# Russoul/cuda-mat

Hardware: AMD Instinct MI355X
Metric: BiCGSTAB iters/sec + SpMV effective HBM GB/s, 10M-row CSR at 1/2/4/8 GPUs (higher is better)
Workload: dtype f64

## Files before the change

cuda_mat_amd/csrc/spmv_pb.h:

```cpp
#pragma once
#include "kernels.h"
#include "valdict.h"

namespace cm {

constexpr int kPbMaxChunks = 16;

struct PbCols {
    int64_t per = 0;
    int chunks = 1;
    int rank = 0;
};

struct PbPlan {
    int n = 0;
    int64_t n_cols = 0;
    int64_t nnz = 0;
    int CB = 0, NCB = 0;
    int64_t per = 0;
    int chunks = 1;
    int64_t chunk_len = 0;
    int bpc = 0;
    int RB = 0, NRB = 0;
    int NW = 0;
    int SR = 0;
    int LPS = 64;
    int depth = 4;
    int NSUB = 0;
    double *pv = nullptr;
    unsigned char *pvi = nullptr;
    const double *dict = nullptr;
    int ndict = 0;
    unsigned short *pc = nullptr;
    unsigned short *pr = nullptr;
    double *P = nullptr;
    int *cstart = nullptr;
    int *col0 = nullptr;
    int *sstart = nullptr;
    int *slen = nullptr;
    int *order = nullptr;
    int part_off[kPbMaxChunks + 2] = {0};
    int placed = -1;
    int place_slabs = 0;
    double place_seconds = 0.0;
    float place_check_ms = 0.f, place_fast_ms = 0.f, place_slow_ms = 0.f;
    char place_classes[192] = {0};
    bool pc_zeroed = false;
    double build_seconds = 0.0;
};

struct PbCut {
    int per, chunks, chunk_len, bpc, CB;
};
struct PbBuild {
    PbPlan p;
    int *bins = nullptr;
    PbCut cut{};
    size_t cap = 0;
    double t0 = 0.0;
    bool verbose = false;
    bool two_pass = false;
    int place = 0;
    bool report_classes = false;
    double place_max_seconds = 0.3;
    int fill_occ = 0;
    int GB = 1, NG = 1;
    unsigned long long *smeta = nullptr;
    int *gstart = nullptr;
};
int pb_build_begin(hipStream_t st, const Config &cfg, int n, int64_t n_cols, int64_t nnz, const int *rp, const int *ci,
                   const PbCols *cols, PbBuild *b);
int pb_build_alloc(hipStream_t st, const Config &cfg, int n, int64_t n_cols, int64_t nnz, const PbCols *cols, PbBuild *b);
int pb_build_count(hipStream_t st, const Config &cfg, const int *rp, const int *ci, PbBuild *b);
int pb_build_values(hipStream_t st, PbBuild *b, const ValDict *vd);
int pb_build_fill(hipStream_t st, PbBuild *b, const int *rp, const int *ci, const double *val, const ValDict *vd, int sub0, int sub1);
int pb_build_end(hipStream_t st, PbBuild *b, PbPlan *out);
void pb_build_abort(PbBuild *b);

bool pb_candidate(hipStream_t st, int n, int64_t n_cols, int64_t nnz, const int *rp, const int *ci);
int pb_build(hipStream_t st, const Config &cfg, int n, int64_t n_cols, int64_t nnz, const int *rp, const int *ci,
             const double *val, PbPlan *out, const PbCols *cols = nullptr, const ValDict *vd = nullptr);
void pb_free(PbPlan *p);
int pb_strict_for(cudamat_ctx *ctx, int *strict);
int launch_spmv_pb(hipStream_t st, const PbPlan &plan, const SpmvArgs &a);
int launch_pb_check(hipStream_t st, const SpmvArgs &a);
int launch_pb_phase1(hipStream_t st, const PbPlan &plan, const SpmvArgs &a, int part);
int launch_pb_phase2(hipStream_t st, const PbPlan &plan, const SpmvArgs &a);

}
```

cuda_mat_amd/csrc/spmv_pb.hip:

```cpp
#include <algorithm>
#include <map>
#include <mutex>
#include <string>
#include <vector>

#include "device.h"
#include "spmv_pb.h"

namespace cm {

typedef unsigned short u16;
constexpr int kPbBuildWaves = 4;
constexpr int kP1Threads = 1024;
constexpr int kP1Unroll = 8;
constexpr int kTileMax = 13312;
constexpr int kPbAlign = 64;

void pb_free(PbPlan *p)
{
    void *ptrs[] = {p->pv, p->pvi, p->pc, p->pr, p->P, p->cstart, p->col0, p->sstart, p->slen, p->order};
    for (void *q : ptrs)
        if (q) CM_DROP(hipFree(q));
    *p = PbPlan();
}

bool pb_candidate(hipStream_t st, int n, int64_t n_cols, int64_t nnz, const int *rp, const int *ci)
{
    (void)st; (void)rp; (void)ci;
    if (n < 65536 || nnz < (1 << 20) || n_cols * 8 < (1 << 20)) return false;
    if ((double)nnz / n < 4.0) return false;
    if ((int64_t)n > (int64_t)kMaxParts * kTileMax) return false;
    return true;
}

__device__ __forceinline__ int col_to_cb(const PbCut &c, int col)
{
    const int q = col / c.per, w = col - q * c.per;
    const int ch = w / c.chunk_len, off = w - ch * c.chunk_len;
    return (q * c.chunks + ch) * c.bpc + off / c.CB;
}

__device__ __forceinline__ int col_to_cb_fast(const PbCut &c, double inv_cb, int col)
{
    if (c.chunks == 1 && col < c.per) {
        int cb = (int)((double)col * inv_cb);
        cb -= (long long)cb * c.CB > (long long)col ? 1 : 0;
        cb += (long long)(cb + 1) * c.CB <= (long long)col ? 1 : 0;
        return cb;
    }
    return col_to_cb(c, col);
}

__device__ __forceinline__ int wave_match_rank(unsigned long long *tab, int key, bool active, int lane, int nkeys, int *count_of_key_lane)
{
    if (lane < nkeys) tab[lane] = 0ULL;
    __builtin_amdgcn_fence(__ATOMIC_RELEASE, "wavefront");
    __builtin_amdgcn_wave_barrier();
    if (active) atomicOr(&tab[key], 1ULL << lane);
    __builtin_amdgcn_fence(__ATOMIC_RELEASE, "wavefront");
    __builtin_amdgcn_wave_barrier();
    const unsigned long long mine = active ? tab[key] : 0ULL;
    *count_of_key_lane = lane < nkeys ? __popcll(tab[lane]) : 0;
    __builtin_amdgcn_fence(__ATOMIC_RELEASE, "wavefront");
    __builtin_amdgcn_wave_barrier();
    return __popcll(mine & ((1ULL << lane) - 1ULL));
}

template <bool FILL>
__global__ __launch_bounds__(64 * kPbBuildWaves) void k_pb_rows(int n, const int *rp, const int *ci,
                                                               const double *val, PbCut cut, const int *col0, int NCB,
                                                               int SR, int NSUB, int *bins, double *pv, u16 *pc, u16 *pr,
                                                               const unsigned char *vidx, unsigned char *pvi, int sub0, int sub1)
{
    extern __shared__ int lds_i[];
    const int wave = threadIdx.x >> 6, lane = threadIdx.x & 63;
    const int sub = sub0 + blockIdx.x * kPbBuildWaves + wave;
    if (sub >= sub1) return;
    int *cur = lds_i + (size_t)wave * NCB;
    for (int c = lane; c < NCB; c += 64) cur[c] = FILL ? bins[(size_t)c * NSUB + sub] : 0;
    __builtin_amdgcn_fence(__ATOMIC_RELEASE, "wavefront");
    __builtin_amdgcn_wave_barrier();
    const long long row0 = (long long)sub * SR;
    const int row1 = (int)(row0 + SR < n ? row0 + SR : n);
    for (int row = (int)row0; row < row1; row++) {
        const int rs = rp[row], re = rp[row + 1];
        for (int k0 = rs; k0 < re; k0 += 64) {
            const int k = k0 + lane;
            const bool active = k < re;
            const int col = active ? ci[k] : -1;
            const int cb = active ? col_to_cb(cut, col) : -1;
            const int prev = __shfl_up(cb, 1, 64);
            const bool head = lane == 0 || cb != prev;
            int hs = head ? lane : 0;
#pragma unroll
            for (int o = 1; o < 64; o <<= 1) {
                const int t = __shfl_up(hs, o, 64);
                if (lane >= o) hs = t > hs ? t : hs;
            }
            const int next = __shfl_down(cb, 1, 64);
            const bool tail = lane == 63 || next != cb;
            if (active) {
                const int base = cur[cb];
                const int rank = lane - hs;
// ... 186 lines not shown
    for (int t0 = 0; t0 < len; t0 += 256) {
        unsigned m[4];
        double v[4];
        unsigned char vi[4];
        int dest[4];
#pragma unroll
        for (int u = 0; u < 4; u++) {
            const int t = t0 + 64 * u + lane;
            const bool active = t < len;
            const int loc = active ? (int)inv[t] : 0;
            m[u] = raw[loc];
            v[u] = 0.0;
            vi[u] = 0;
            if (active) { if (pvi) vi[u] = sval8[start + loc]; else v[u] = sval[start + loc]; }
            const int cbl = active ? (int)cbs[loc] : 0;
            dest[u] = __shfl(gdst, cbl, 64) + (t - __shfl(lbase, cbl, 64));
        }
#pragma unroll
        for (int u = 0; u < 4; u++) {
            if (t0 + 64 * u + lane < len) {
                if (pvi) pvi[dest[u]] = vi[u];
                else pv[dest[u]] = v[u];
                pc[dest[u]] = (u16)((m[u] >> 16) & 0xffff);
                pr[dest[u]] = (u16)(m[u] & 0xffff);
            }
        }
    }
}

__global__ __launch_bounds__(kBlock) void k_pb_colsum(int NSUB, const int *bins, int *colsum)
{
    __shared__ int red[kBlock / 64];
    const int *b = bins + (size_t)blockIdx.x * NSUB;
    int acc = 0;
    for (int i = threadIdx.x; i < NSUB; i += kBlock) acc += b[i];
#pragma unroll
    for (int o = 32; o > 0; o >>= 1) acc += __shfl_xor(acc, o, 64);
    if ((threadIdx.x & 63) == 0) red[threadIdx.x >> 6] = acc;
    __syncthreads();
    if (threadIdx.x == 0) {
        int t = 0;
        for (int w = 0; w < kBlock / 64; w++) t += red[w];
        colsum[blockIdx.x] = t;
    }
}

__global__ __launch_bounds__(kBlock) void k_pb_colscan(int NCB, const int *colsum, int *cstart, int align)
{
    __shared__ int lds_waves[kBlock / 64];
    int run = 0;
    for (int c0 = 0; c0 < NCB; c0 += kBlock) {
        const int c = c0 + threadIdx.x;
        const int v = c < NCB ? (colsum[c] + align - 1) / align * align : 0;
        int total;
        const int ex = block_scan_int(v, lds_waves, &total);
        if (c < NCB) cstart[c] = run + ex;
        run += total;
    }
    if (threadIdx.x == 0) cstart[NCB] = run;
}

__global__ __launch_bounds__(kBlock) void k_pb_segscan(int NCB, int NSUB, const int *cstart, int *bins, int *sstart,
                                                       int *slen)
{
    __shared__ int lds_waves[kBlock / 64];
    const int c = blockIdx.x;
    int *b = bins + (size_t)c * NSUB;
    int run = cstart[c];
    for (int s0 = 0; s0 < NSUB; s0 += kBlock) {
        const int sidx = s0 + threadIdx.x;
        const int cnt = sidx < NSUB ? b[sidx] : 0;
        int total;
        const int ex = block_scan_int(cnt, lds_waves, &total);
        if (sidx < NSUB) {
            const int start = run + ex;
            b[sidx] = start;
            sstart[(size_t)sidx * NCB + c] = start;
            slen[(size_t)sidx * NCB + c] = cnt;
        }
        run += total;
    }
}

static int round_blocks(int64_t n, int tile_max)
{
    int64_t m = (n + (int64_t)256 * tile_max - 1) / ((int64_t)256 * tile_max);
    if (m < 1) m = 1;
    return (int)(256 * m);
}

static void pb_scratch_free(PbBuild *b)
{
    if (b->smeta) CM_DROP(hipFree(b->smeta));
    if (b->gstart) CM_DROP(hipFree(b->gstart));
    b->smeta = nullptr;
    b->gstart = nullptr;
}

void pb_build_abort(PbBuild *b)
{
    pb_scratch_free(b);
    if (b->bins) CM_DROP(hipFree(b->bins));
    b->bins = nullptr;
    pb_free(&b->p);
}

int pb_build_begin(hipStream_t st, const Config &cfg, int n, int64_t n_cols, int64_t nnz, const int *rp, const int *ci,
                   const PbCols *cols, PbBuild *b)
{
    CM_TRY(pb_build_alloc(st, cfg, n, n_cols, nnz, cols, b));
    return pb_build_count(st, cfg, rp, ci, b);
}

int pb_build_alloc(hipStream_t st, const Config &cfg, int n, int64_t n_cols, int64_t nnz, const PbCols *cols, PbBuild *b)
{
    b->t0 = now_s();
    PbPlan &p = b->p;
    p = PbPlan();
    p.n = n;
    p.n_cols = n_cols;
    p.nnz = nnz;
    int local_slice = 0;
    if (cols && cols->per > 0 && cols->per < n_cols) {
        p.per = cols->per;
        p.chunks = cols->chunks < 1 ? 1 : cols->chunks > kPbMaxChunks ? kPbMaxChunks : cols->chunks;
        p.chunk_len = (p.per + p.chunks - 1) / p.chunks;
        p.bpc = (int)((p.chunk_len + kTileMax - 1) / kTileMax);
        p.CB = (int)((p.chunk_len + p.bpc - 1) / p.bpc);
        const int64_t slices = (n_cols + p.per - 1) / p.per;
        p.NCB = (int)(slices * p.chunks * p.bpc);
        local_slice = cols->rank;
    } else {
        p.per = n_cols;
        p.chunks = 1;
        p.chunk_len = n_cols;
        p.NCB = round_blocks(n_cols, kTileMax);
        p.CB = (int)((n_cols + p.NCB - 1) / p.NCB);
        p.NCB = (int)((n_cols + p.CB - 1) / p.CB);
        p.bpc = p.NCB;
    }
    const double seg_target = 48.0;
    double nsub_t = (double)nnz / ((double)p.NCB * seg_target);
    const bool few = nsub_t < 2560.0 && (double)n / 2048.0 * 8.0 * 8.0 <= 144.0 * 1024.0;
    double min_waves = few ? 2048.0 : 4096.0;
    if (cfg.pb_min_waves) min_waves = (double)cfg.pb_min_waves;
    if (nsub_t < min_waves) nsub_t = min_waves;
    if (nsub_t > (double)n / 16.0) nsub_t = (double)n / 16.0;
    if (nsub_t < 4.0) nsub_t = 4.0;
    p.NW = nsub_t >= 4096.0 ? 16 : nsub_t >= 2048.0 ? 8 : 4;
    int nrb = (int)(nsub_t / p.NW / 256.0 + 0.5) * 256;
    if (nrb < 256) nrb = 256;
    const int nrb_min = (int)(((int64_t)n + kTileMax - 1) / kTileMax);
    while (nrb < nrb_min) nrb += 256;
    if (nrb > kMaxParts) nrb = kMaxParts;
    p.NRB = nrb;
    p.RB = (int)(((int64_t)n + p.NRB - 1) / p.NRB);
    p.SR = (p.RB + p.NW - 1) / p.NW;
    if (p.SR < 1) p.SR = 1;
    p.RB = p.SR * p.NW;
    p.NRB = (int)(((int64_t)n + p.RB - 1) / p.RB);
    p.NSUB = p.NRB * p.NW;
    const double seg = (double)nnz / ((double)p.NCB * p.NSUB);
    p.LPS = seg <= 6.0 ? 16 : seg <= 22.0 ? 32 : 64;
    p.depth = few ? 16 : 4;
    if (cfg.pb_depth) p.depth = cfg.pb_depth;
    if (p.NRB > kMaxParts || p.CB > 65536 || p.SR > 65536 || (size_t)p.RB * 8 > 150 * 1024 ||
        sizeof(int) * (size_t)kPbBuildWaves * p.NCB > 150 * 1024) {
        set_error("pb_build: matrix shape outside the blocked kernel's limits");
        return CUDAMAT_ERR_ARG;
    }
    const size_t nbins = (size_t)p.NCB * p.NSUB;
    int *&bins = b->bins;
    bins = nullptr;
    int rc = CUDAMAT_OK;
    do {
        if ((rc = dev_alloc(&bins, nbins))) break;
        constexpr int align = kPbAlign;
        const size_t cap = (size_t)nnz + (size_t)(align - 1) * (size_t)p.NCB + 16;
        b->cap = cap;
        if ((rc = dev_alloc(&p.cstart, (size_t)p.NCB + 1))) break;
        if ((rc = dev_alloc(&p.col0, (size_t)p.NCB + 1))) break;
        if ((rc = dev_alloc(&p.order, (size_t)p.NCB))) break;
        {
            std::vector<int> h0((size_t)p.NCB + 1), ord;
            const int per_slice = p.chunks * p.bpc;
            for (int cb = 0; cb <= p.NCB; cb++) {
                const int64_t q = cb / per_slice, ch = (cb % per_slice) / p.bpc, k = cb % p.bpc;
                int64_t in_piece = k * (int64_t)p.CB;
                if (in_piece > p.chunk_len) in_piece = p.chunk_len;
                int64_t in_slice = ch * p.chunk_len + in_piece;
                if (in_slice > p.per) in_slice = p.per;
                int64_t c0 = q * p.per + in_slice;
                if (c0 > n_cols) c0 = n_cols;
                h0[(size_t)cb] = (int)c0;
            }
            ord.reserve((size_t)p.NCB);
            const int slices = p.NCB / per_slice;
            if (slices > 1) {
                for (int k = 0; k < per_slice; k++) ord.push_back(local_slice * per_slice + k);
                p.part_off[0] = 0;
                p.part_off[1] = (int)ord.size();
                for (int ch = 0; ch < p.chunks; ch++) {
                    for (int q = 0; q < slices; q++)
                        if (q != local_slice)
                            for (int k = 0; k < p.bpc; k++) ord.push_back((q * p.chunks + ch) * p.bpc + k);
                    p.part_off[ch + 2] = (int)ord.size();
                }
            } else {
                for (int cb = 0; cb < p.NCB; cb++) ord.push_back(cb);
                p.part_off[0] = 0;
                for (int ch = 0; ch <= p.chunks; ch++) p.part_off[ch + 1] = p.NCB;
            }
            if (hipMemcpyAsync(p.col0, h0.data(), sizeof(int) * h0.size(), hipMemcpyHostToDevice, st) != hipSuccess ||
                hipMemcpyAsync(p.order, ord.data(), sizeof(int) * ord.size(), hipMemcpyHostToDevice, st) != hipSuccess ||
                hipStreamSynchronize(st) != hipSuccess) { rc = CUDAMAT_ERR_HIP; set_error("pb column cut upload failed"); break; }
        }
        b->cut = PbCut{(int)p.per, p.chunks, (int)p.chunk_len, p.bpc, p.CB};
        if ((rc = dev_alloc(&p.sstart, nbins))) break;
        if ((rc = dev_alloc(&p.slen, nbins))) break;
        if ((rc = set_max_lds((const void *)k_pb_count))) break;
        if ((rc = set_max_lds((const void *)k_pb_rows<true>))) break;
        b->GB = 1;
        while (b->GB * kPbGroups < p.NCB) b->GB *= 2;
        b->NG = (p.NCB + b->GB - 1) / b->GB;
        b->fill_occ = cfg.pb_fill_occ;
        b->place = cfg.pb_place;
        b->place_max_seconds = 1e-3 * cfg.pb_place_max_ms;
        b->verbose = cfg.verbose != 0;
        b->report_classes = cfg.verbose >= 2;
        b->two_pass = cfg.pb_fill2 != 0 && nnz > 0 && nnz < 0x7fffffffLL && p.SR <= 65536 && b->GB <= 64;
        if (b->two_pass) {
            if (dev_alloc(&b->smeta, (size_t)nnz) != CUDAMAT_OK || dev_alloc(&b->gstart, (size_t)p.NSUB * (size_t)(b->NG + 1)) != CUDAMAT_OK) {
                if (b->smeta) CM_DROP(hipFree(b->smeta));
                b->smeta = nullptr;
                b->two_pass = false;
            }
        }
    } while (0);
    if (rc) pb_build_abort(b);
    return rc;
}

int pb_build_count(hipStream_t st, const Config &cfg, const int *rp, const int *ci, PbBuild *b)
{
    PbPlan &p = b->p;
    const int n = p.n;
    const int64_t nnz = p.nnz;
    int *bins = b->bins;
    constexpr int align = kPbAlign;
    int rc = CUDAMAT_OK;
    do {
        const PbCut cut = b->cut;
        const unsigned grid = (unsigned)((p.NSUB + kPbBuildWaves - 1) / kPbBuildWaves);
        const size_t lds = sizeof(int) * (size_t)kPbBuildWaves * p.NCB;
        hipLaunchKernelGGL(k_pb_count, dim3(grid), dim3(64 * kPbBuildWaves), lds, st, n, rp, ci, cut, p.NCB, p.SR, p.NSUB, bins, 0, p.NSUB);
        if (hipGetLastError() != hipSuccess) { rc = CUDAMAT_ERR_HIP; set_error("pb count launch failed"); break; }
        hipLaunchKernelGGL(k_pb_colsum, dim3(p.NCB), dim3(kBlock), 0, st, p.NSUB, bins, p.cstart);
        hipLaunchKernelGGL(k_pb_colscan, dim3(1), dim3(kBlock), 0, st, p.NCB, p.cstart, p.cstart, align);
        hipLaunchKernelGGL(k_pb_segscan, dim3(p.NCB), dim3(kBlock), 0, st, p.NCB, p.NSUB, p.cstart, bins, p.sstart, p.slen);
        int counted = -1;
        if (hipGetLastError() != hipSuccess ||
            hipMemcpyAsync(&counted, p.cstart + p.NCB, sizeof(int), hipMemcpyDeviceToHost, st) != hipSuccess ||
            hipStreamSynchronize(st) != hipSuccess) { rc = CUDAMAT_ERR_HIP; set_error("pb scan failed"); break; }
        if ((int64_t)counted < nnz || (int64_t)counted > nnz + (int64_t)(align - 1) * p.NCB) {
            rc = CUDAMAT_ERR_ARG; set_error("pb_build: counted %d entries, expected %lld", counted, (long long)nnz); break;
        }
        b->verbose = cfg.verbose != 0;
        b->report_classes = cfg.verbose >= 2;
    } while (0);
    if (rc) pb_build_abort(b);
    return rc;
}

__global__ __launch_bounds__(1024) void k_place_probe(const double2 *rd, double2 *wr, long n2)
{
    const long per = (n2 + gridDim.x - 1) / gridDim.x;
    const long lo = blockIdx.x * per, hi = lo + per < n2 ? lo + per : n2;
    for (long i = lo + threadIdx.x; i < hi; i += 1024) {
        const double2 v = rd[i];
        double2 o;
        o.x = v.x * 1.5;
        o.y = v.y + 1.0;
        wr[i] = o;
    }
}

struct PlaceTimer {
    hipStream_t st;
    hipEvent_t e0 = nullptr, e1 = nullptr;
    bool ok = false;
    int launches = 0;
    explicit PlaceTimer(hipStream_t s) : st(s) { ok = hipEventCreate(&e0) == hipSuccess && hipEventCreate(&e1) == hipSuccess; }
    ~PlaceTimer()
    {
        if (e0) CM_DROP(hipEventDestroy(e0));
        if (e1) CM_DROP(hipEventDestroy(e1));
    }
    float ms(const void *rd, void *wr, size_t bytes)
    {
        float t[12];
        int n = 0;
        while (ok && n < 12) {
            if (hipEventRecord(e0, st) != hipSuccess) { ok = false; break; }
            hipLaunchKernelGGL(k_place_probe, dim3(256), dim3(1024), 0, st, (const double2 *)rd, (double2 *)wr, (long)(bytes / 16));
            float x = 0.f;
            if (hipGetLastError() != hipSuccess || hipEventRecord(e1, st) != hipSuccess || hipEventSynchronize(e1) != hipSuccess ||
                hipEventElapsedTime(&x, e0, e1) != hipSuccess) { ok = false; break; }
            launches++;
            t[n++] = x;
            if (n >= 3) {
                const float lo = fminf(t[n - 1], fminf(t[n - 2], t[n - 3])), hi = fmaxf(t[n - 1], fmaxf(t[n - 2], t[n - 3]));
                if (hi <= 1.015f * lo) return lo;
            }
        }
        if (!ok || n < 3) return -1.f;
        return fminf(t[n - 1], fminf(t[n - 2], t[n - 3]));
    }
};

constexpr size_t kPlaceBlock = (size_t)2 << 30;
constexpr size_t kPlaceSample = (size_t)896 << 20;
constexpr size_t kPlaceSlab = (size_t)16 << 30;
constexpr size_t kPlaceMinBytes = (size_t)2 << 30;
constexpr size_t kPlaceMaxHeld = (size_t)96 << 30;
constexpr float kPlaceGap = 1.035f;

struct PlaceMemo {
    unsigned gen = ~0u;
    std::map<char *, int> cls;
    std::vector<char *> ref;
    float t_own = 0.f;
    float t_lo = 0.f, t_hi = 0.f;
    std::vector<std::pair<char *, float>> provisional;
    bool relabel = false;
    void reset() { cls.clear(); ref.clear(); provisional.clear(); t_own = t_lo = t_hi = 0.f; relabel = false; }
};
static std::mutex g_place_mu;
static std::map<int, PlaceMemo> g_place;

struct PlaceRun { size_t slab; size_t first, count; int cls; };

struct PlaceSlab {
// ... 247 lines not shown
        }
        hipLaunchKernelGGL(k_pb_group, dim3(grid), dim3(64 * kPbBuildWaves), pad, st, p.n, rp, ci, val, vidx, b->cut, p.col0, p.NCB, p.SR,
                           p.slen, b->GB, b->NG, b->gstart, p.P, p.pvi ? (unsigned char *)p.P : (unsigned char *)nullptr, b->smeta, sub0, sub1);
        const long long buckets = (long long)(sub1 - sub0) * b->NG;
        hipLaunchKernelGGL(k_pb_scatter, dim3((unsigned)((buckets + kPbScatterWaves - 1) / kPbScatterWaves)), dim3(64 * kPbScatterWaves), 0, st,
                           p.NCB, p.NSUB, p.slen, b->bins, b->GB, b->NG, b->gstart, p.P, p.pvi ? (const unsigned char *)p.P : (const unsigned char *)nullptr,
                           b->smeta, p.pv, p.pvi, p.pc, p.pr, sub0, sub1);
    } else {
        const size_t lds = sizeof(int) * (size_t)kPbBuildWaves * p.NCB;
        hipLaunchKernelGGL(k_pb_rows<true>, dim3(grid), dim3(64 * kPbBuildWaves), lds, st, p.n, rp, ci, val, b->cut, p.col0,
                           p.NCB, p.SR, p.NSUB, b->bins, p.pv, p.pc, p.pr, vidx, p.pvi, sub0, sub1);
    }
    if (hipGetLastError() != hipSuccess) { set_error("pb fill launch failed"); pb_build_abort(b); return CUDAMAT_ERR_HIP; }
    return CUDAMAT_OK;
}

static void pb_print_plan(const PbPlan &p)
{
    const size_t nbins = (size_t)p.NCB * p.NSUB;
    std::vector<int> hl(nbins);
    if (hipMemcpy(hl.data(), p.slen, sizeof(int) * nbins, hipMemcpyDeviceToHost) != hipSuccess) return;
    long long hist[7] = {0, 0, 0, 0, 0, 0, 0}, in_long = 0;
    for (int v : hl) {
        hist[v == 0 ? 0 : v <= 8 ? 1 : v <= 24 ? 2 : v <= 48 ? 3 : v <= 64 ? 4 : v <= 128 ? 5 : 6]++;
        if (v > 64) in_long += v;
    }
    fprintf(stderr, "[cudamat] pb arrays: pv %p pvi %p pc %p pr %p P %p sstart %p slen %p cstart %p\n", (void *)p.pv, (void *)p.pvi, (void *)p.pc,
            (void *)p.pr, (void *)p.P, (void *)p.sstart, (void *)p.slen, (void *)p.cstart);
    fprintf(stderr, "[cudamat] pb plan: %d x %lld, nnz %lld, NCB %d (CB %d), NSUB %d (NW %d, SR %d), LPS %d, depth %d; segments: "
                    "empty %lld, 1-8 %lld, 9-24 %lld, 25-48 %lld, 49-64 %lld, 65-128 %lld, >128 %lld; %.1f %% of the entries in "
                    "segments longer than a wave\n",
            p.n, (long long)p.n_cols, (long long)p.nnz, p.NCB, p.CB, p.NSUB, p.NW, p.SR, p.LPS, p.depth, hist[0], hist[1], hist[2], hist[3],
            hist[4], hist[5], hist[6], 100.0 * (double)in_long / (double)(p.nnz > 0 ? p.nnz : 1));
}

static void place_report_classes(hipStream_t st, const PbPlan &p, size_t cap)
{
    if (!pool_enabled()) return;
    PlaceTimer tm(st);
    if (!tm.ok) return;
    int dev = 0;
    if (hipGetDevice(&dev) != hipSuccess) return;
    std::lock_guard<std::mutex> lock(g_place_mu);
    PlaceMemo &m = g_place[dev];
    if (m.gen != pool_generation()) { m.gen = pool_generation(); m.reset(); }
    std::vector<char *> slabs;
    std::vector<char *> scratch(3, nullptr);
    for (int k = 0; k < 4 && !(scratch[0] && scratch[1] && scratch[2]); k++) {
        char *base = nullptr;
        if (hipMalloc(&base, kPlaceSlab) != hipSuccess) { CM_DROP(hipGetLastError()); break; }
        slabs.push_back(base);
        char *seg = nullptr;
        size_t bytes = 0;
        if (!pool_segment_of(base, &seg, &bytes)) break;
        char *b0 = seg + ((size_t)(base - seg) + kPlaceBlock - 1) / kPlaceBlock * kPlaceBlock;
        for (char *q = b0; q + kPlaceBlock <= base + bytes; q += kPlaceBlock) {
            const int c = place_class_of(tm, m, q);
            if (c >= 0 && c < 3 && !scratch[c]) scratch[c] = q;
        }
    }
    struct Arr { const char *name; const char *ptr; size_t bytes; };
    const Arr arrs[4] = {{"values", p.pv ? (const char *)p.pv : (const char *)p.pvi, p.pv ? sizeof(double) * cap : cap},
                         {"col idx", (const char *)p.pc, sizeof(u16) * cap}, {"row idx", (const char *)p.pr, sizeof(u16) * cap}, {"products", (const char *)p.P, sizeof(double) * cap}};
    for (const Arr &a : arrs) {
        std::string line;
        for (size_t off = 0; off + kPlaceSample <= a.bytes; off += kPlaceSample) {
            int cls = -1;
            float worst = 0.f;
            for (int k = 0; k < 3; k++) {
                if (!scratch[k]) continue;
                const float t = tm.ms(a.ptr + off, scratch[k] + kPlaceBlock - kPlaceSample, kPlaceSample);
                if (t > worst) { worst = t; cls = k; }
            }
            line += cls < 0 || !(m.t_hi >= kPlaceGap * m.t_lo) || worst <= sqrtf(m.t_lo * m.t_hi) ? '?' : (char)('0' + cls);
        }
        fprintf(stderr, "[cudamat] pb classes: %-8s at %p, per %zu MB: %s\n", a.name, (const void *)a.ptr, kPlaceSample >> 20, line.c_str());
    }
    for (char *q : slabs) CM_DROP(hipFree(q));
}

int pb_build_end(hipStream_t st, PbBuild *b, PbPlan *out)
{
    if (hipStreamSynchronize(st) != hipSuccess) { set_error("pb fill failed"); pb_build_abort(b); return CUDAMAT_ERR_HIP; }
    if (b->verbose) pb_print_plan(b->p);
    if (b->report_classes && sizeof(double) * b->cap >= kPlaceMinBytes) place_report_classes(st, b->p, b->cap);
    pb_scratch_free(b);
    CM_DROP(hipFree(b->bins));
    b->bins = nullptr;
    b->p.build_seconds = now_s() - b->t0;
    *out = b->p;
    b->p = PbPlan();
    return CUDAMAT_OK;
}

int pb_build(hipStream_t st, const Config &cfg, int n, int64_t n_cols, int64_t nnz, const int *rp, const int *ci,
             const double *val, PbPlan *out, const PbCols *cols, const ValDict *vd)
{
    PbBuild b;
    CM_TRY(pb_build_begin(st, cfg, n, n_cols, nnz, rp, ci, cols, &b));
    CM_TRY(pb_build_values(st, &b, vd));
    CM_TRY(pb_build_fill(st, &b, rp, ci, val, vd, 0, b.p.NSUB));
    return pb_build_end(st, &b, out);
}


__global__ __launch_bounds__(kP1Threads) void k_pb_phase1(const double *x, const int *col0, const int *list,
                                                          const int *cstart, const double *pv, const u16 *pc,
                                                          double *P, const LoopState *st, int cb0)
{
    extern __shared__ __attribute__((aligned(16))) double xs[];
    if (st && st->state != 0) return;
    const int cb = list ? list[blockIdx.x] : (int)blockIdx.x + cb0;
    const int s = cstart[cb], e = cstart[cb + 1];
    if (s >= e) return;
    const int c0 = col0[cb], cn = col0[cb + 1] - c0;
    for (int i = threadIdx.x; i < cn; i += kP1Threads) xs[i] = x[c0 + i];
    __syncthreads();
    constexpr int STEP = 2 * kP1Threads;
    const int k0 = (s & ~1) + 2 * (int)threadIdx.x;
    for (int k = k0; k < e; k += 4 * STEP) {
        double2 v[4];
        ushort2 c[4];
        bool full[4];
#pragma unroll
        for (int u = 0; u < 4; u++) {
            const int kk = k + u * STEP;
            full[u] = kk >= s && kk + 1 < e;
            if (full[u]) {
                v[u] = *(const double2 *)(pv + kk);
                c[u] = *(const ushort2 *)(pc + kk);
            }
        }
#pragma unroll
        for (int u = 0; u < 4; u++) {
            const int kk = k + u * STEP;
            if (full[u]) {
                double2 o;
                o.x = v[u].x * xs[c[u].x];
                o.y = v[u].y * xs[c[u].y];
                *(double2 *)(P + kk) = o;
            } else {
                if (kk >= s && kk < e) P[kk] = pv[kk] * xs[pc[kk]];
                if (kk + 1 >= s && kk + 1 < e) P[kk + 1] = pv[kk + 1] * xs[pc[kk + 1]];
            }
        }
    }
}

__global__ __launch_bounds__(kP1Threads) void k_pb_phase1_dict(const double *x, const int *col0, const int *list,
                                                               const int *cstart, const unsigned char *pvi, const u16 *pc,
                                                               const double *dict, int cb_doubles, double *P,
                                                               const LoopState *st, int cb0)
{
    extern __shared__ __attribute__((aligned(16))) double xs[];
    if (st && st->state != 0) return;
    const int cb = list ? list[blockIdx.x] : (int)blockIdx.x + cb0;
    const int s = cstart[cb], e = cstart[cb + 1];
    if (s == e) return;
    double *dv = xs + cb_doubles;
    const int c0 = col0[cb], cn = col0[cb + 1] - c0;
    for (int i = threadIdx.x; i < cn; i += kP1Threads) xs[i] = x[c0 + i];
    if (threadIdx.x < kDictMax) dv[threadIdx.x] = dict[threadIdx.x];
    __syncthreads();
    constexpr int U = kP1Unroll, STEP = 2 * kP1Threads, CH = U * STEP;
    const int a0 = (s + 1) & ~1;
    if (threadIdx.x == 0 && s < a0) P[s] = dv[pvi[s]] * xs[pc[s]];
    int kb = a0;
    const int t2 = 2 * (int)threadIdx.x;
    for (; kb + CH <= e; kb += CH) {
        const int k = kb + t2;
        u16 iv[U];
        unsigned cv[U];
#pragma unroll
        for (int u = 0; u < U; u++) {
            iv[u] = *(const u16 *)(pvi + k + u * STEP);
            cv[u] = *(const unsigned *)(pc + k + u * STEP);
        }
#pragma unroll
        for (int u = 0; u < U; u++) {
            double2 o;
            o.x = dv[iv[u] & 0xffu] * xs[cv[u] & 0xffffu];
            o.y = dv[iv[u] >> 8] * xs[cv[u] >> 16];
            *(double2 *)(P + k + u * STEP) = o;
        }
    }
    {
        const int m = e > kb ? (e - kb) / STEP : 0;
        const int k = kb + t2;
        u16 iv[U - 1];
        unsigned cv[U - 1];
#pragma unroll
        for (int u = 0; u < U - 1; u++) {
            if (u < m) {
                iv[u] = *(const u16 *)(pvi + k + u * STEP);
                cv[u] = *(const unsigned *)(pc + k + u * STEP);
            }
        }
#pragma unroll
        for (int u = 0; u < U - 1; u++) {
            if (u < m) {
                double2 o;
                o.x = dv[iv[u] & 0xffu] * xs[cv[u] & 0xffffu];
                o.y = dv[iv[u] >> 8] * xs[cv[u] >> 16];
                *(double2 *)(P + k + u * STEP) = o;
            }
        }
        const int kr = k + m * STEP;
        if (kr + 1 < e) {
            const u16 iw = *(const u16 *)(pvi + kr);
            const unsigned cw = *(const unsigned *)(pc + kr);
            double2 o;
            o.x = dv[iw & 0xffu] * xs[cw & 0xffffu];
            o.y = dv[iw >> 8] * xs[cw >> 16];
            *(double2 *)(P + kr) = o;
        } else if (kr < e) {
            P[kr] = dv[pvi[kr]] * xs[pc[kr]];
        }
    }
}

struct Pb2Args {
    int n, NCB, SR;
    const int *sstart, *slen;
    const double *P;
    const u16 *pr;
    const double *d, *xd;
    double alpha, beta;
    double *y;
    int dot;
    const double *w;
    double *parts;
    const LoopState *st;
    int strict;
    const int *xd_idx;
};

__device__ __forceinline__ void pb_seg_add(double *my, int r, double p, bool on, int lane, int group_first, bool strict)
{
    if (!strict) {
        if (on) unsafeAtomicAdd(&my[r], p);
        return;
    }
    const int r_prev = __shfl_up(r, 1, 64);
    const int on_prev = __shfl_up((int)on, 1, 64);
    const bool d1 = on && lane > group_first && on_prev && r_prev == r;
    if (on && !d1) unsafeAtomicAdd(&my[r], p);
    if (__ballot(d1) == 0) return;
    const bool d2 = d1 && __shfl_up((int)d1, 1, 64) != 0;
    if (d1 && !d2) unsafeAtomicAdd(&my[r], p);
    if (__ballot(d2) == 0) return;
    int head = d1 ? 0 : lane;
#pragma unroll
    for (int o = 1; o < 64; o <<= 1) {
        const int t = __shfl_up(head, o, 64);
        if (lane >= o) head = t > head ? t : head;
    }
    const int rank = on ? lane - head : 0;
    for (int q = 2; __ballot(on && rank >= q); q++)
        if (on && rank == q) unsafeAtomicAdd(&my[r], p);
}

__global__ __launch_bounds__(64) void k_lds_order_probe(int *mismatch)
{
    __shared__ double acc[64], val[64], start[64];
    const int lane = threadIdx.x;
    unsigned long long z = 0x9E3779B97F4A7C15ULL * (unsigned long long)(lane + 1);
    int bad = 0;
    for (int pat = 0; pat < 4; pat++) {
        const int addr = pat == 0 ? 0 : pat == 1 ? lane >> 3 : pat == 2 ? (lane & 31) : (lane & 3);
        const int naddr = pat == 0 ? 1 : pat == 1 ? 8 : pat == 2 ? 32 : 4;
        for (int rep = 0; rep < 4; rep++) {
            z ^= z >> 30; z *= 0xBF58476D1CE4E5B9ULL; z ^= z >> 27; z *= 0x94D049BB133111EBULL; z ^= z >> 31;
            const double v = 0.5 + (double)(z >> 11) * 0x1.0p-53;
            const double c = 3.0 + (double)((z * 0x9E3779B97F4A7C15ULL) >> 11) * 0x1.0p-53;
            val[lane] = v;
            start[lane] = c;
            acc[lane] = c;
            __syncthreads();
            unsafeAtomicAdd(&acc[addr], v);
            __syncthreads();
            if (lane < naddr) {
#pragma clang fp contract(off)
                double e = start[lane];
                for (int l = 0; l < 64; l++) {
                    const int al = pat == 0 ? 0 : pat == 1 ? l >> 3 : pat == 2 ? (l & 31) : (l & 3);
                    if (al == lane) e = e + val[l];
                }
                if (__double_as_longlong(e) != __double_as_longlong(acc[lane])) bad = 1;
            }
            __syncthreads();
        }
    }
    if (bad) atomicOr(mismatch, 1);
}

int pb_strict_for(cudamat_ctx *ctx, int *strict)
{
    *strict = 1;
    if (ctx->cfg.pb_strict) return CUDAMAT_OK;
    if (ctx->lds_lane_order < 0) {
        int *flag = (int *)ctx->scratch.get(), h = 1;
        CM_HIP(hipMemsetAsync(flag, 0, sizeof(int), ctx->stream));
        hipLaunchKernelGGL(k_lds_order_probe, dim3(1), dim3(64), 0, ctx->stream, flag);
        CM_HIP(hipGetLastError());
        CM_HIP(hipMemcpyAsync(&h, flag, sizeof(int), hipMemcpyDeviceToHost, ctx->stream));
        CM_HIP(hipStreamSynchronize(ctx->stream));
        if (ctx->cfg.pb_probe_fail) h = 1;
        ctx->lds_lane_order = h ? 0 : 1;
        if (h || ctx->cfg.verbose)
            fprintf(stderr, "[cudamat] LDS order probe: equal addresses of one ds_add_f64 are %s -> blocked SpMV phase 2 in its %s form\n",
                    h ? (ctx->cfg.pb_probe_fail ? "reported NOT in lane order (PB_PROBE_FAIL)" : "NOT served in lane order")
                      : "served in lane order", h ? "architected-order (PB_STRICT)" : "default");
    }
    *strict = ctx->lds_lane_order ? 0 : 1;
    return CUDAMAT_OK;
}

template <int NW, int LPS, int DEPTH, bool IDX = false>
__global__ __launch_bounds__(64 * NW) void k_pb_phase2(Pb2Args a)
{
    extern __shared__ __attribute__((aligned(16))) double yt[];
    if (a.st && a.st->state != 0) return;
    const int wave = threadIdx.x >> 6, lane = threadIdx.x & 63;
    const int sub = blockIdx.x * NW + wave;
    double *my = yt + (size_t)wave * a.SR;
    for (int i = lane; i < a.SR; i += 64) my[i] = 0.0;
    __builtin_amdgcn_fence(__ATOMIC_RELEASE, "wavefront");
    __builtin_amdgcn_wave_barrier();
    const int *ss = a.sstart + (size_t)sub * a.NCB;
    const int *sl = a.slen + (size_t)sub * a.NCB;
    for (int cb0 = 0; cb0 < a.NCB; cb0 += 64) {
        const int c = cb0 + lane;
        const int mys = c < a.NCB ? ss[c] : 0;
        const int myl = c < a.NCB ? sl[c] : 0;
        const int lim = a.NCB - cb0 < 64 ? a.NCB - cb0 : 64;
        const bool grouped = LPS < 64 && !__any(myl > LPS);
        if (!grouped) {
            for (int j = 0; j < lim; j += DEPTH) {
                int s[DEPTH], l[DEPTH];
                double pv4[DEPTH];
                int r4[DEPTH];
#pragma unroll
                for (int u = 0; u < DEPTH; u++) {
                    s[u] = __builtin_amdgcn_readlane(mys, (j + u) & 63);
                    l[u] = __builtin_amdgcn_readlane(myl, (j + u) & 63);
                }
#pragma unroll
                for (int u = 0; u < DEPTH; u++) {
                    const bool on = lane < l[u];
                    pv4[u] = on ? a.P[s[u] + lane] : 0.0;
                    r4[u] = on ? (int)a.pr[s[u] + lane] : 0;
                }
#pragma unroll
                for (int u = 0; u < DEPTH; u++) {
                    pb_seg_add(my, r4[u], pv4[u], lane < l[u], lane, 0, a.strict != 0);
                    for (int off0 = 64; off0 < l[u]; off0 += 64) {
                        const int off = off0 + lane;
                        const bool on = off < l[u];
                        pb_seg_add(my, on ? (int)a.pr[s[u] + off] : 0, on ? a.P[s[u] + off] : 0.0, on, lane, 0, a.strict != 0);
                    }
                }
            }
        } else {
            constexpr int G = 64 / LPS;
            const int g = lane / LPS, li = lane % LPS;
            for (int j = 0; j < lim; j += DEPTH * G) {
                int s[DEPTH], l[DEPTH];
                double pv4[DEPTH];
                int r4[DEPTH];
#pragma unroll
                for (int u = 0; u < DEPTH; u++) {
                    const int cbi = j + u * G + g;
                    s[u] = __shfl(mys, cbi & 63, 64);
                    l[u] = cbi < 64 ? __shfl(myl, cbi & 63, 64) : 0;
                }
#pragma unroll
                for (int u = 0; u < DEPTH; u++) {
                    const bool on = li < l[u];
                    pv4[u] = on ? a.P[s[u] + li] : 0.0;
                    r4[u] = on ? (int)a.pr[s[u] + li] : 0;
                }
#pragma unroll
                for (int u = 0; u < DEPTH; u++) {
                    if (!a.strict) {
                        if (li < l[u]) unsafeAtomicAdd(&my[r4[u]], pv4[u]);
                    } else {
#pragma unroll
                        for (int gg = 0; gg < G; gg++)
                            pb_seg_add(my, r4[u], pv4[u], g == gg && li < l[u], lane, gg * LPS, true);
                    }
                }
            }
        }
    }
    __builtin_amdgcn_fence(__ATOMIC_RELEASE, "wavefront");
    __builtin_amdgcn_wave_barrier();
    double acc0 = 0.0, acc1 = 0.0;
    const long long row0 = (long long)sub * a.SR;
    for (int i = lane; i < a.SR && row0 + i < a.n; i += 64) {
#pragma clang fp contract(off)
        const int row = (int)(row0 + i);
        double sum = my[i];
        if (a.d) {
            const double dx = a.d[row] * a.xd[IDX ? a.xd_idx[row] : row];
            sum = sum + dx;
        }
        double out = a.alpha * sum;
        if (a.beta != 0.0) {
            const double by = a.beta * a.y[row];
            out = out + by;
        }
        a.y[row] = out;
        if (a.dot) {
            acc0 += out * a.w[row];
            acc1 += out * out;
        }
    }
    if (a.dot) {
        double *red = yt + (size_t)NW * a.SR;
#pragma unroll
        for (int o = 32; o > 0; o >>= 1) {
            acc0 += __shfl_xor(acc0, o, 64);
            acc1 += __shfl_xor(acc1, o, 64);
        }
        if (lane == 0) {
            red[2 * wave] = acc0;
            red[2 * wave + 1] = acc1;
        }
        __syncthreads();
        if (threadIdx.x == 0) {
            double t0 = 0.0, t1 = 0.0;
            for (int q = 0; q < NW; q++) {
                t0 += red[2 * q];
                t1 += red[2 * q + 1];
            }
            a.parts[2 * blockIdx.x] = t0;
            a.parts[2 * blockIdx.x + 1] = t1;
        }
    }
}

int launch_pb_check(hipStream_t st, const SpmvArgs &a)
{
    if (a.loop.st && a.check == CHECK_HALF) CM_TRY(launch_check(st, a.loop, a.half, CHECK_HALF));
    return CUDAMAT_OK;
}

static int launch_pb_phase1_blocks(hipStream_t st, const PbPlan &p, const SpmvArgs &a, const int *list, int first, int last)
{
    if (last <= first) return CUDAMAT_OK;
    if (p.pvi) {
        CM_TRY(set_max_lds((const void *)k_pb_phase1_dict));
        const int cbd = (p.CB + 1) & ~1;
        hipLaunchKernelGGL(k_pb_phase1_dict, dim3(last - first), dim3(kP1Threads), sizeof(double) * (size_t)(cbd + kDictMax), st, a.x,
                           p.col0, list ? list + first : (const int *)nullptr, p.cstart, p.pvi, p.pc, p.dict, cbd, p.P, a.loop.st,
                           list ? 0 : first);
        CM_HIP(hipGetLastError());
        return CUDAMAT_OK;
    }
    CM_TRY(set_max_lds((const void *)k_pb_phase1));
    hipLaunchKernelGGL(k_pb_phase1, dim3(last - first), dim3(kP1Threads), sizeof(double) * (size_t)p.CB, st, a.x, p.col0,
                       list ? list + first : (const int *)nullptr, p.cstart, p.pv, p.pc, p.P, a.loop.st, list ? 0 : first);
    CM_HIP(hipGetLastError());
    return CUDAMAT_OK;
}

int launch_pb_phase1(hipStream_t st, const PbPlan &p, const SpmvArgs &a, int part)
{
    if (part < 0) return launch_pb_phase1_blocks(st, p, a, nullptr, 0, p.NCB);
    return launch_pb_phase1_blocks(st, p, a, p.order, p.part_off[part], p.part_off[part + 1]);
}

int launch_spmv_pb(hipStream_t st, const PbPlan &p, const SpmvArgs &a)
{
    CM_TRY(launch_pb_check(st, a));
    CM_TRY(launch_pb_phase1(st, p, a, -1));
    return launch_pb_phase2(st, p, a);
}

int launch_pb_phase2(hipStream_t st, const PbPlan &p, const SpmvArgs &a)
{
    Pb2Args b;
    b.n = p.n; b.NCB = p.NCB; b.SR = p.SR;
    b.sstart = p.sstart; b.slen = p.slen;
    b.P = p.P; b.pr = p.pr;
    b.d = a.d; b.xd = a.xd; b.xd_idx = a.xd_idx;
    b.alpha = a.alpha; b.beta = a.beta;
    b.y = a.y; b.dot = a.dot; b.w = a.w; b.parts = a.parts;
    b.st = a.loop.st;
    b.strict = a.pb_strict;
    const size_t lds = sizeof(double) * ((size_t)p.NW * p.SR + 2 * (size_t)p.NW);
    const bool idx = b.d && b.xd_idx;
#define CM_P2D(NWV, LPSV, DV, IDXV)                                                                               \
    do {                                                                                                          \
        CM_TRY(set_max_lds((const void *)k_pb_phase2<NWV, LPSV, DV, IDXV>));                                     \
        hipLaunchKernelGGL((k_pb_phase2<NWV, LPSV, DV, IDXV>), dim3(p.NRB), dim3(64 * NWV), lds, st, b);         \
    } while (0)
#define CM_P2(NWV, LPSV)                                                                                  \
    do {                                                                                                  \
        if (idx && p.depth >= 16) CM_P2D(NWV, LPSV, 16, true);                                            \
        else if (idx) CM_P2D(NWV, LPSV, 4, true);                                                         \
        else if (p.depth >= 16) CM_P2D(NWV, LPSV, 16, false);                                             \
        else if (p.depth >= 8) CM_P2D(NWV, LPSV, 8, false);                                               \
        else CM_P2D(NWV, LPSV, 4, false);                                                                 \
    } while (0)
#define CM_P2_LPS(NWV)                                           \
    do {                                                         \
        if (p.LPS == 16) CM_P2(NWV, 16);                         \
        else if (p.LPS == 32) CM_P2(NWV, 32);                    \
        else CM_P2(NWV, 64);                                     \
    } while (0)
    switch (p.NW) {
    case 4:  CM_P2_LPS(4); break;
    case 8:  CM_P2_LPS(8); break;
    default: CM_P2_LPS(16); break;
    }
#undef CM_P2_LPS
#undef CM_P2
#undef CM_P2D
    CM_HIP(hipGetLastError());
    return CUDAMAT_OK;
}

}
```

Measured before the change: 184.0.

## Reorder partial-product row indices into per-row-slab contiguous layout

After the build, the u16 row-index array is permuted so that each row slab's entries sit contiguously in column-block order, with a new per-slab rstart offset. Phase 2 then streams the row indices sequentially from that offset, using a DPP prefix scan of segment lengths for the packed-lane path, instead of gathering them from the column-major layout. The aim is more coalesced and sequential reads of the row indices in the reduce phase. It costs an extra device buffer and copy at build time, and it assumes every other consumer of pr, such as phase 1 writes or placement, is fine with the new ordering.

```diff
diff --git a/cuda_mat_amd/csrc/spmv_pb.h b/cuda_mat_amd/csrc/spmv_pb.h
--- a/cuda_mat_amd/csrc/spmv_pb.h
+++ b/cuda_mat_amd/csrc/spmv_pb.h
@@ -38,6 +38,7 @@
     int *col0 = nullptr;
     int *sstart = nullptr;
     int *slen = nullptr;
+    int *rstart = nullptr;
     int *order = nullptr;
     int part_off[kPbMaxChunks + 2] = {0};
     int placed = -1;
diff --git a/cuda_mat_amd/csrc/spmv_pb.hip b/cuda_mat_amd/csrc/spmv_pb.hip
--- a/cuda_mat_amd/csrc/spmv_pb.hip
+++ b/cuda_mat_amd/csrc/spmv_pb.hip
@@ -18,7 +18,7 @@
 
 void pb_free(PbPlan *p)
 {
-    void *ptrs[] = {p->pv, p->pvi, p->pc, p->pr, p->P, p->cstart, p->col0, p->sstart, p->slen, p->order};
+    void *ptrs[] = {p->pv, p->pvi, p->pc, p->pr, p->P, p->cstart, p->col0, p->sstart, p->slen, p->rstart, p->order};
     for (void *q : ptrs)
         if (q) CM_DROP(hipFree(q));
     *p = PbPlan();
@@ -371,6 +371,49 @@
     }
 }
 
+__global__ __launch_bounds__(kBlock) void k_pb_rstart(int n, const int *rp, int SR, int NSUB, int *rstart)
+{
+    const int sub = blockIdx.x * kBlock + threadIdx.x;
+    if (sub > NSUB) return;
+    const long long row0 = (long long)sub * SR;
+    rstart[sub] = rp[row0 < n ? row0 : n] - rp[0];
+}
+
+constexpr int kPbMoveDepth = 8;
+__global__ __launch_bounds__(64 * kPbBuildWaves) void k_pb_rows_by_wave(int NCB, int NSUB, const int *sstart, const int *slen,
+                                                                       const int *rstart, const u16 *src, u16 *dst)
+{
+    const int wave = threadIdx.x >> 6, lane = threadIdx.x & 63;
+    const int sub = blockIdx.x * kPbBuildWaves + wave;
+    if (sub >= NSUB) return;
+    const int *ss = sstart + (size_t)sub * NCB;
+    const int *sl = slen + (size_t)sub * NCB;
+    u16 *out = dst + rstart[sub];
+    int run = 0;
+    for (int cb0 = 0; cb0 < NCB; cb0 += 64) {
+        const int c = cb0 + lane;
+        const int mys = c < NCB ? ss[c] : 0;
+        const int myl = c < NCB ? sl[c] : 0;
+        for (int j = 0; j < 64; j += kPbMoveDepth) {
+            int s[kPbMoveDepth], l[kPbMoveDepth];
+            u16 r[kPbMoveDepth];
+#pragma unroll
+            for (int u = 0; u < kPbMoveDepth; u++) {
+                s[u] = __builtin_amdgcn_readlane(mys, (j + u) & 63);
+                l[u] = __builtin_amdgcn_readlane(myl, (j + u) & 63);
+            }
+#pragma unroll
+            for (int u = 0; u < kPbMoveDepth; u++) r[u] = lane < l[u] ? src[s[u] + lane] : (u16)0;
+#pragma unroll
+            for (int u = 0; u < kPbMoveDepth; u++) {
+                if (lane < l[u]) out[run + lane] = r[u];
+                for (int off = 64 + lane; off < l[u]; off += 64) out[run + off] = src[s[u] + off];
+                run += l[u];
+            }
+        }
+    }
+}
+
 static int round_blocks(int64_t n, int tile_max)
 {
     int64_t m = (n + (int64_t)256 * tile_max - 1) / ((int64_t)256 * tile_max);
@@ -468,6 +511,7 @@
         const size_t cap = (size_t)nnz + (size_t)(align - 1) * (size_t)p.NCB + 16;
         b->cap = cap;
         if ((rc = dev_alloc(&p.cstart, (size_t)p.NCB + 1))) break;
+        if ((rc = dev_alloc(&p.rstart, (size_t)p.NSUB + 1))) break;
         if ((rc = dev_alloc(&p.col0, (size_t)p.NCB + 1))) break;
         if ((rc = dev_alloc(&p.order, (size_t)p.NCB))) break;
         {
@@ -547,6 +591,7 @@
         hipLaunchKernelGGL(k_pb_colsum, dim3(p.NCB), dim3(kBlock), 0, st, p.NSUB, bins, p.cstart);
         hipLaunchKernelGGL(k_pb_colscan, dim3(1), dim3(kBlock), 0, st, p.NCB, p.cstart, p.cstart, align);
         hipLaunchKernelGGL(k_pb_segscan, dim3(p.NCB), dim3(kBlock), 0, st, p.NCB, p.NSUB, p.cstart, bins, p.sstart, p.slen);
+        hipLaunchKernelGGL(k_pb_rstart, dim3((unsigned)(p.NSUB / kBlock + 1)), dim3(kBlock), 0, st, n, rp, p.SR, p.NSUB, p.rstart);
         int counted = -1;
         if (hipGetLastError() != hipSuccess ||
             hipMemcpyAsync(&counted, p.cstart + p.NCB, sizeof(int), hipMemcpyDeviceToHost, st) != hipSuccess ||
@@ -960,6 +1005,22 @@
 int pb_build_end(hipStream_t st, PbBuild *b, PbPlan *out)
 {
     if (hipStreamSynchronize(st) != hipSuccess) { set_error("pb fill failed"); pb_build_abort(b); return CUDAMAT_ERR_HIP; }
+    {
+        PbPlan &p = b->p;
+        DevBuf<u16> old;
+        int rc = old.alloc(b->cap);
+        if (!rc && hipMemcpyAsync(old, p.pr, sizeof(u16) * b->cap, hipMemcpyDeviceToDevice, st) != hipSuccess) rc = CUDAMAT_ERR_HIP;
+        if (!rc) {
+            hipLaunchKernelGGL(k_pb_rows_by_wave, dim3((unsigned)((p.NSUB + kPbBuildWaves - 1) / kPbBuildWaves)), dim3(64 * kPbBuildWaves), 0, st,
+                               p.NCB, p.NSUB, p.sstart, p.slen, p.rstart, old, p.pr);
+            if (hipGetLastError() != hipSuccess || hipStreamSynchronize(st) != hipSuccess) rc = CUDAMAT_ERR_HIP;
+        }
+        if (rc) {
+            if (rc == CUDAMAT_ERR_HIP) set_error("pb row-index reordering failed");
+            pb_build_abort(b);
+            return rc;
+        }
+    }
     if (b->verbose) pb_print_plan(b->p);
     if (b->report_classes && sizeof(double) * b->cap >= kPlaceMinBytes) place_report_classes(st, b->p, b->cap);
     pb_scratch_free(b);
@@ -1099,7 +1160,7 @@
 
 struct Pb2Args {
     int n, NCB, SR;
-    const int *sstart, *slen;
+    const int *sstart, *slen, *rstart;
     const double *P;
     const u16 *pr;
     const double *d, *xd;
@@ -1194,19 +1255,34 @@
     return CUDAMAT_OK;
 }
 
+__device__ __forceinline__ int wave_scan_rows_dpp(int v, int lane)
+{
+    v += __builtin_amdgcn_update_dpp(0, v, 0x111, 0xf, 0xf, true);
+    v += __builtin_amdgcn_update_dpp(0, v, 0x112, 0xf, 0xf, true);
+    v += __builtin_amdgcn_update_dpp(0, v, 0x114, 0xf, 0xf, true);
+    v += __builtin_amdgcn_update_dpp(0, v, 0x118, 0xf, 0xf, true);
+    const int t0 = __builtin_amdgcn_readlane(v, 15), t1 = __builtin_amdgcn_readlane(v, 31), t2 = __builtin_amdgcn_readlane(v, 47);
+    return v + (lane >= 16 ? t0 : 0) + (lane >= 32 ? t1 : 0) + (lane >= 48 ? t2 : 0);
+}
+
 template <int NW, int LPS, int DEPTH, bool IDX = false>
 __global__ __launch_bounds__(64 * NW) void k_pb_phase2(Pb2Args a)
 {
     extern __shared__ __attribute__((aligned(16))) double yt[];
-    if (a.st && a.st->state != 0) return;
     const int wave = threadIdx.x >> 6, lane = threadIdx.x & 63;
     const int sub = blockIdx.x * NW + wave;
+    const int state = a.st ? a.st->state : 0;
+    const int run0 = a.rstart[__builtin_amdgcn_readfirstlane(sub)];
+    __asm__ volatile("" : : "s"(run0), "s"(state));
+    if (state != 0) return;
     double *my = yt + (size_t)wave * a.SR;
     for (int i = lane; i < a.SR; i += 64) my[i] = 0.0;
     __builtin_amdgcn_fence(__ATOMIC_RELEASE, "wavefront");
     __builtin_amdgcn_wave_barrier();
     const int *ss = a.sstart + (size_t)sub * a.NCB;
     const int *sl = a.slen + (size_t)sub * a.NCB;
+    const u16 *prw = a.pr + run0;
+    int run = 0;
     for (int cb0 = 0; cb0 < a.NCB; cb0 += 64) {
         const int c = cb0 + lane;
         const int mys = c < a.NCB ? ss[c] : 0;
@@ -1223,11 +1299,14 @@
                     s[u] = __builtin_amdgcn_readlane(mys, (j + u) & 63);
                     l[u] = __builtin_amdgcn_readlane(myl, (j + u) & 63);
                 }
+                int start = run;
+                __asm__ volatile("" : "+s"(start));
 #pragma unroll
                 for (int u = 0; u < DEPTH; u++) {
                     const bool on = lane < l[u];
                     pv4[u] = on ? a.P[s[u] + lane] : 0.0;
-                    r4[u] = on ? (int)a.pr[s[u] + lane] : 0;
+                    r4[u] = on ? (int)prw[run + lane] : 0;
+                    run += l[u];
                 }
 #pragma unroll
                 for (int u = 0; u < DEPTH; u++) {
@@ -1235,40 +1314,45 @@
                     for (int off0 = 64; off0 < l[u]; off0 += 64) {
                         const int off = off0 + lane;
                         const bool on = off < l[u];
-                        pb_seg_add(my, on ? (int)a.pr[s[u] + off] : 0, on ? a.P[s[u] + off] : 0.0, on, lane, 0, a.strict != 0);
+                        pb_seg_add(my, on ? (int)prw[start + off] : 0, on ? a.P[s[u] + off] : 0.0, on, lane, 0, a.strict != 0);
                     }
+                    start += l[u];
                 }
             }
         } else {
             constexpr int G = 64 / LPS;
             const int g = lane / LPS, li = lane % LPS;
+            const int inc = wave_scan_rows_dpp(myl, lane);
+            const int total = __builtin_amdgcn_readlane(inc, 63);
+            const int mypk = ((inc - myl) << 6) | myl;
             for (int j = 0; j < lim; j += DEPTH * G) {
-                int s[DEPTH], l[DEPTH];
+                int s[DEPTH], pk[DEPTH];
                 double pv4[DEPTH];
                 int r4[DEPTH];
 #pragma unroll
                 for (int u = 0; u < DEPTH; u++) {
                     const int cbi = j + u * G + g;
                     s[u] = __shfl(mys, cbi & 63, 64);
-                    l[u] = cbi < 64 ? __shfl(myl, cbi & 63, 64) : 0;
+                    pk[u] = cbi < 64 ? __shfl(mypk, cbi & 63, 64) : 0;
                 }
 #pragma unroll
                 for (int u = 0; u < DEPTH; u++) {
-                    const bool on = li < l[u];
+                    const bool on = li < (pk[u] & 63);
                     pv4[u] = on ? a.P[s[u] + li] : 0.0;
-                    r4[u] = on ? (int)a.pr[s[u] + li] : 0;
+                    r4[u] = on ? (int)prw[run + (pk[u] >> 6) + li] : 0;
                 }
 #pragma unroll
                 for (int u = 0; u < DEPTH; u++) {
                     if (!a.strict) {
-                        if (li < l[u]) unsafeAtomicAdd(&my[r4[u]], pv4[u]);
+                        if (li < (pk[u] & 63)) unsafeAtomicAdd(&my[r4[u]], pv4[u]);
                     } else {
 #pragma unroll
                         for (int gg = 0; gg < G; gg++)
-                            pb_seg_add(my, r4[u], pv4[u], g == gg && li < l[u], lane, gg * LPS, true);
+                            pb_seg_add(my, r4[u], pv4[u], g == gg && li < (pk[u] & 63), lane, gg * LPS, true);
                     }
                 }
             }
+            run += total;
         }
     }
     __builtin_amdgcn_fence(__ATOMIC_RELEASE, "wavefront");
@@ -1360,7 +1444,7 @@
 {
     Pb2Args b;
     b.n = p.n; b.NCB = p.NCB; b.SR = p.SR;
-    b.sstart = p.sstart; b.slen = p.slen;
+    b.sstart = p.sstart; b.slen = p.slen; b.rstart = p.rstart;
     b.P = p.P; b.pr = p.pr;
     b.d = a.d; b.xd = a.xd; b.xd_idx = a.xd_idx;
     b.alpha = a.alpha; b.beta = a.beta;
```

Result: no change. 183.9 (-0.1%).
